# rbesenczi/newMSM

Hardware: AMD Instinct MI355X
Metric: label-cost evals/sec (higher is better)
Workload: dtype f64; 1 GPU; pairwise sulc (D=1) unary label-cost table, ico6 data grid / ico4 control grid, 19 labels, 48678 evals = 3187573 point samples per step (BASELINE config 2); kind=univariate, simmeasure=correlation, replicas=1

## Files before the change

### include/msmhip.h

```cpp
#ifndef MSMHIP_H
#define MSMHIP_H

#include <stddef.h>
#include <stdint.h>

#ifdef __cplusplus
extern "C" {
#endif

#define MSM_ABI_VERSION 12

#define MSM_OK 0
#define MSM_ERR_INVALID (-1)
#define MSM_ERR_HIP (-2)
#define MSM_ERR_OUTSIDE (-3)
#define MSM_ERR_NOTFOUND (-4)
#define MSM_ERR_NOGPU (-5)
#define MSM_ERR_STATE (-6)
#define MSM_ERR_CAPACITY (-7)
#define MSM_ERR_ROTATION (-8)

#define MSM_RAD 100.0
#define MSM_FOLDING 1e7

// ... 3 lines not shown

int         msm_abi_version(void);
const char *msm_last_error(void);
int         msm_device_count(void);

int msm_icosphere_counts(int order, int32_t *V, int32_t *T);
int msm_icosphere(int order, double radius, double *xyz, int32_t *tri);
int msm_mesh_adjacency(const int32_t *tri, int32_t V, int32_t T, int32_t *nbr_ptr, int32_t *nbr, int32_t *tid_ptr, int32_t *tid);
int msm_vertex_areas(const double *xyz, const int32_t *tri, int32_t V, int32_t T, double *area);
int msm_resample_anatomy_grid(const double *cp_xyz, int32_t N, const int32_t *cp_tri, int32_t Tc, int32_t levels, double rad, int32_t *Va, int32_t *Ta,
                              double *axyz, int32_t *atri, int32_t *w_ptr, int32_t *w_cp, double *w_val, int32_t *face_ptr, int32_t *face_idx);
int msm_cp_spacings(const double *xyz, const int32_t *tri, int32_t V, int32_t T, double *maxsep, double *mvdmax);
int msm_label_sampling_grid(int sg_order, double max_dist, int abs_is_int, int32_t cap,
                            double *samples, int32_t *nsamples, double *barycentres, int32_t *nbarycentres);
int msm_rescale_sampling_grid(const double *samples, int32_t n, double *scale, double *labels);
int msm_rotation_matrix(const double ci[3], const double index[3], double R[9]);
int msm_cp_rotations(const double centre[3], const double *cp_xyz, int32_t N, double *rot);
int msm_estimate_triplets(const int32_t *tri, int32_t T, int32_t *triplets);
int msm_estimate_pairs(const int32_t *tri, int32_t V, int32_t T, int32_t *pairs);
int msm_octree_signature(const double *xyz, const int32_t *tri, int32_t V, int32_t T, int64_t stats[5], uint64_t *signature);
int msm_ray_table_check(const double *xyz, const int32_t *tri, int32_t V, int32_t T, int32_t nsamples, uint64_t seed, int64_t report[10]);
int msm_ray_hint_check(const double *xyz, const int32_t *tri, int32_t V, int32_t T, int32_t nsamples, uint64_t seed, int64_t report[8], int32_t *cells,
                       int64_t cells_cap);

msm_ctx *msm_ctx_create(int device);
msm_ctx *msm_ctx_create_on_stream(int device, void *hip_stream);
void     msm_ctx_destroy(msm_ctx *ctx);
int      msm_ctx_synchronize(msm_ctx *ctx);
void    *msm_ctx_stream(msm_ctx *ctx);
void     msm_store_release_i64(int64_t *addr, int64_t value);
int64_t  msm_load_acquire_i64(const int64_t *addr);
int64_t  msm_min_acquire_i64(const int64_t *addr, int32_t n);
int      msm_ctx_wait_stream(msm_ctx *ctx, void *hip_stream);
int      msm_ctx_staging_stats(msm_ctx *ctx, int64_t out[4]);
int      msm_ctx_time_queries(msm_ctx *ctx, int enable);
int      msm_ctx_query_kernel_ms(msm_ctx *ctx, double *ms);
int      msm_query_lanes(int64_t n_queries);
void    *msm_host_alloc(msm_ctx *ctx, size_t bytes);
void     msm_host_free(msm_ctx *ctx, void *p);
int      msm_host_register(msm_ctx *ctx, void *p, size_t bytes);

msm_mesh *msm_mesh_create(msm_ctx *ctx, const double *xyz, int32_t V, const int32_t *tri, int32_t T);
void      msm_mesh_destroy(msm_mesh *m);
int       msm_mesh_update_coords(msm_mesh *m, const double *xyz);
int       msm_mesh_get_coords(msm_mesh *m, double *xyz);
int       msm_mesh_set_features(msm_mesh *m, const double *feat, int32_t D);
// ... 80 lines not shown
int msm_cost_patches(msm_cost *c, int32_t *ngroups, int32_t *ptr, int32_t *idx, int64_t cap);
int msm_cost_absolute_weights(msm_cost *c, double *absw );
int msm_cost_unary_table(msm_cost *c, double *U);
int msm_cost_unary_table_async(msm_cost *c);
int msm_cost_unary_table_fetch(msm_cost *c, double *U);
int msm_cost_unary_batch(msm_cost *c, const int32_t *nodes, const int32_t *labels, int32_t n, double *out);
int msm_cost_triplet_batch(msm_cost *c, const int32_t *triplet, const int32_t *la, const int32_t *lb, const int32_t *lc, int32_t n, double *out);
int msm_cost_triplet_octets(msm_cost *c, const int32_t *labeling, int32_t label, double *E);
int msm_cost_triplet_octets_prefetch(msm_cost *c, const int32_t *labeling, int32_t label, double *E);
int msm_cost_prefetch_stats(msm_cost *c, int64_t *taken, int64_t *dropped);
int msm_cost_pairwise_batch(msm_cost *c, const int32_t *pair, const int32_t *la, const int32_t *lb, int32_t n, double *out);
int msm_cost_pairwise_table(msm_cost *c, double *paircosts);
int msm_cost_triplet_table(msm_cost *c, int32_t t0, int32_t t1, double *tcosts);
int msm_cost_total(msm_cost *c, const int32_t *labeling, double *total, double parts[3]);
int msm_cost_enable_timing(msm_cost *c, int enable);
int msm_cost_kernel_times(msm_cost *c, double *ms, int32_t cap, int32_t *n);
int msm_cost_counters(msm_cost *c, int64_t counters[4]);
#define MSM_ROUTE_UNARY 0
#define MSM_ROUTE_MOVE 1
#define MSM_ROUTE_MOVE_NBLK 2
#define MSM_ROUTE_MOVE_CAP 3
#define MSM_ROUTE_MOVE_MAXTRI 4
#define MSM_ROUTE_MOVE_TAILS 5
#define MSM_UNARY_NONE 0
#define MSM_UNARY_UNIVARIATE 1
#define MSM_UNARY_FLAT 2
#define MSM_UNARY_FEATURES 3
#define MSM_UNARY_MV8 4
#define MSM_UNARY_PW8_4 5
#define MSM_UNARY_PW8_8 6
#define MSM_MOVE_NONE 0
#define MSM_MOVE_FUSED_0 1
#define MSM_MOVE_FUSED_1 2
#define MSM_MOVE_FUSED_2 3
#define MSM_MOVE_FUSED_3 4
#define MSM_MOVE_OCTETS_SAMPLE 5
#define MSM_MOVE_OCTETS_SAMPLE_MV8 6
#define MSM_MOVE_OCTETS_HO 7
#define MSM_MOVE_STRAIN 8
int msm_cost_routes(msm_cost *c, int32_t routes[8]);

typedef struct msm_group msm_group;
typedef struct msm_group_params {
    int32_t simmeasure;
    int32_t fixnan;
    double  lambda, mu, kappa, k_exp, rexp, range;
// ... 75 lines not shown
```

### newmsm_amd/_lib.py

```python
import ctypes as C
import os

_HERE = os.path.dirname(os.path.abspath(__file__))
LIB_PATH = os.environ.get("MSM_LIB_PATH") or os.path.join(_HERE, "libmsmhip.so")

c_dp = C.POINTER(C.c_double)
c_ip = C.POINTER(C.c_int32)
c_lp = C.POINTER(C.c_int64)

MSM_OK = 0
ERR_NAMES = {-1: "MSM_ERR_INVALID", -2: "MSM_ERR_HIP", -3: "MSM_ERR_OUTSIDE", -4: "MSM_ERR_NOTFOUND", -5: "MSM_ERR_NOGPU",
             -6: "MSM_ERR_STATE", -7: "MSM_ERR_CAPACITY", -8: "MSM_ERR_ROTATION"}


class MsmError(RuntimeError):

    def __init__(self, code, message):
        super().__init__("%s (%d): %s" % (ERR_NAMES.get(code, "MSM_ERR"), code, message))
        self.code = code


class GroupParams(C.Structure):
    _fields_ = [("simmeasure", C.c_int32), ("fixnan", C.c_int32), ("lambda_", C.c_double), ("mu", C.c_double),
                ("kappa", C.c_double), ("k_exp", C.c_double), ("rexp", C.c_double), ("range", C.c_double), ("percentile", C.c_double)]
# ... 5 lines not shown
                ("rexp", C.c_double), ("range", C.c_double), ("percentile", C.c_double)]


_VP = C.c_void_p
SIGNATURES = {
    "msm_abi_version": (C.c_int, []),
    "msm_last_error": (C.c_char_p, []),
    "msm_device_count": (C.c_int, []),
    "msm_icosphere_counts": (C.c_int, [C.c_int, c_ip, c_ip]),
    "msm_icosphere": (C.c_int, [C.c_int, C.c_double, c_dp, c_ip]),
    "msm_mesh_adjacency": (C.c_int, [c_ip, C.c_int32, C.c_int32, c_ip, c_ip, c_ip, c_ip]),
    "msm_vertex_areas": (C.c_int, [c_dp, c_ip, C.c_int32, C.c_int32, c_dp]),
    "msm_resample_anatomy_grid": (C.c_int, [c_dp, C.c_int32, c_ip, C.c_int32, C.c_int32, C.c_double, c_ip, c_ip, c_dp, c_ip, c_ip, c_ip, c_dp, c_ip, c_ip]),
    "msm_cp_spacings": (C.c_int, [c_dp, c_ip, C.c_int32, C.c_int32, c_dp, c_dp]),
    "msm_label_sampling_grid": (C.c_int, [C.c_int, C.c_double, C.c_int, C.c_int32, c_dp, c_ip, c_dp, c_ip]),
    "msm_rescale_sampling_grid": (C.c_int, [c_dp, C.c_int32, c_dp, c_dp]),
    "msm_rotation_matrix": (C.c_int, [c_dp, c_dp, c_dp]),
    "msm_cp_rotations": (C.c_int, [c_dp, c_dp, C.c_int32, c_dp]),
    "msm_estimate_triplets": (C.c_int, [c_ip, C.c_int32, c_ip]),
    "msm_estimate_pairs": (C.c_int, [c_ip, C.c_int32, C.c_int32, c_ip]),
    "msm_octree_signature": (C.c_int, [c_dp, c_ip, C.c_int32, C.c_int32, C.POINTER(C.c_int64), C.POINTER(C.c_uint64)]),
    "msm_ray_table_check": (C.c_int, [c_dp, c_ip, C.c_int32, C.c_int32, C.c_int32, C.c_uint64, C.POINTER(C.c_int64)]),
    "msm_ray_hint_check": (C.c_int, [c_dp, c_ip, C.c_int32, C.c_int32, C.c_int32, C.c_uint64, C.POINTER(C.c_int64), c_ip, C.c_int64]),
    "msm_ctx_create": (_VP, [C.c_int]),
    "msm_ctx_create_on_stream": (_VP, [C.c_int, _VP]),
    "msm_ctx_destroy": (None, [_VP]),
    "msm_ctx_synchronize": (C.c_int, [_VP]),
    "msm_ctx_stream": (_VP, [_VP]),
    "msm_store_release_i64": (None, [_VP, C.c_int64]),
    "msm_load_acquire_i64": (C.c_int64, [_VP]),
    "msm_min_acquire_i64": (C.c_int64, [_VP, C.c_int32]),
    "msm_ctx_time_queries": (C.c_int, [_VP, C.c_int]),
    "msm_ctx_query_kernel_ms": (C.c_int, [_VP, c_dp]),
    "msm_query_lanes": (C.c_int, [C.c_int64]),
    "msm_group_context": (_VP, [_VP]),
    "msm_ctx_wait_stream": (C.c_int, [_VP, _VP]),
    "msm_ctx_staging_stats": (C.c_int, [_VP, C.POINTER(C.c_int64)]),
    "msm_host_alloc": (_VP, [_VP, C.c_size_t]),
    "msm_host_free": (None, [_VP, _VP]),
    "msm_host_register": (C.c_int, [_VP, _VP, C.c_size_t]),
    "msm_mesh_create": (_VP, [_VP, c_dp, C.c_int32, c_ip, C.c_int32]),
    "msm_mesh_destroy": (None, [_VP]),
    "msm_mesh_update_coords": (C.c_int, [_VP, c_dp]),
    "msm_mesh_get_coords": (C.c_int, [_VP, c_dp]),
    "msm_mesh_set_features": (C.c_int, [_VP, c_dp, C.c_int32]),
    "msm_mesh_sizes": (C.c_int, [_VP, c_ip, c_ip, c_ip]),
# ... 134 lines not shown
```

### newmsm_amd/api.py

```python
import ctypes as C

import numpy as np

from ._lib import CostParams, MsmError, c_dp, c_ip, c_lp, check, lib

WEIGHTS_PROJECTED = 0
WEIGHTS_RAW = 1
KINDS = dict(univariate=0, multivariate=1, patchwise=2, ho_univariate=3, ho_multivariate=4)


def _soa(points):
    a = np.ascontiguousarray(np.asarray(points, dtype=np.float64).reshape(-1, 3).T)
    return a, a.ctypes.data_as(c_dp)


def _aos(soa, n):
    return np.ascontiguousarray(np.asarray(soa).reshape(3, n).T)


def _tri_soa(tri):
    a = np.ascontiguousarray(np.asarray(tri, dtype=np.int32).reshape(-1, 3).T)
    return a, a.ctypes.data_as(c_ip)


# ... 767 lines not shown
        check(lib().msm_cost_total(self.h, pl, C.byref(tot), parts.ctypes.data_as(c_dp)))
        return tot.value, parts

    def enable_timing(self, on=True):
        check(lib().msm_cost_enable_timing(self.h, int(on)))

    def kernel_times(self):
        ms = np.zeros(64)
        n = C.c_int32()
        check(lib().msm_cost_kernel_times(self.h, ms.ctypes.data_as(c_dp), 64, C.byref(n)))
        return ms[: n.value].copy()

    def counters(self):
        c = (C.c_int64 * 4)()
        check(lib().msm_cost_counters(self.h, c))
        return dict(samples=c[0], unary=c[1], triplet=c[2], pairwise=c[3])

    UNARY_ROUTES = ("none", "univariate", "flat", "features", "mv8", "pw8<4>", "pw8<8>")
    MOVE_ROUTES = ("none", "fused0", "fused1", "fused2", "fused3", "octets_sample", "octets_sample_mv8", "octets_ho", "strain")

    def routes(self):
        r = (C.c_int32 * 8)()
        check(lib().msm_cost_routes(self.h, r))
        return dict(unary=self.UNARY_ROUTES[r[0]], move=self.MOVE_ROUTES[r[1]], move_nblk=r[2], move_cap=r[3], move_maxtri=r[4], move_tails=r[5])


class DiscreteGroupCostFunction:

    def __init__(self, ctx, num_subjects, simmeasure=2, fixnan=False, lambda_=0.1, mu=0.1, kappa=10.0, k_exp=2.0, rexp=2.0, range_=1.0,
                 percentile=0.75):
        from ._lib import GroupParams

        self.ctx = ctx
        self.S = num_subjects
        self.params = GroupParams(simmeasure, int(fixnan), lambda_, mu, kappa, k_exp, rexp, range_, percentile)
        self.h = lib().msm_group_create(ctx.h, C.byref(self.params), num_subjects)
        if not self.h:
            raise MsmError(-1, lib().msm_last_error().decode())
        self._keep = {}

    def close(self):
        if getattr(self, "h", None) and getattr(self.ctx, "h", None):
            lib().msm_group_destroy(self.h)
        self.h = None

    def __del__(self):
        self.close()
# ... 224 lines not shown
```

### newmsm_amd/csrc/cost.cpp

```cpp
#include <algorithm>
#include <chrono>
#include <cmath>
#include <cstdio>
#include <cstdlib>
#include <cstring>

#include "cost_internal.hpp"
#include "host_parallel.hpp"

using namespace msm;

namespace msm {
int ensure_vertex_major(msm_cost *c) {
    if (c->vm_valid) return MSM_OK;
    msm_ctx *ctx = c->ctx;
    const int Ns = c->source->V, D = c->D, R = c->cfw_rows;
    std::vector<double> vm((size_t)Ns * D);
    for (int d = 0; d < D; ++d)
        for (int v = 0; v < Ns; ++v) vm[(size_t)v * D + d] = c->sfeat[(size_t)d * Ns + v];
    MSM_HIP(c->d_sfeat_vm.ensure(vm.size()));
    {
        const int st = upload_staged(ctx, c->d_sfeat_vm.p, vm.data(), sizeof(double) * vm.size());
        if (st) return st;
    }
// ... 175 lines not shown
    u.tfeat = c->target->d_feat.p;
    u.D = c->D;
    u.N = N;
    u.L = c->L;
    u.cp = c->cpgrid->d_xyz.p;
    st = ensure_label_rotations(c);
    if (st) return st;
    u.rnl = c->d_rnl.p;
    u.labels = c->d_labels.p;
    u.src = c->source->d_xyz.p;
    u.Nsrc = c->source->V;
    u.sfeat = c->d_sfeat.p;
    u.cfw = c->cfw.empty() ? nullptr : c->d_cfw.p;
    u.cfw_rows = c->cfw_rows;
    u.pptr = c->d_pptr.p;
    u.pidx = c->d_pidx.p;
    u.order = c->d_order.p;
    u.absw = c->d_absw.p;
    u.pmax = c->pmax;
    u.simmeasure = c->p.simmeasure;
    u.percentile = c->p.percentile;
    u.U = c->d_U.p;
    const size_t nsamp = (size_t)c->L * c->pidx.size();
    MSM_HIP(c->d_tval.ensure(nsamp));
    MSM_HIP(c->d_fix_list.ensure(nsamp));
    MSM_HIP(c->d_fix_pt.ensure(3 * nsamp));
    if (!c->d_fix_count.p) MSM_HIP(c->d_fix_count.zero(unary_fix_counter_words(), ctx->stream));
    if (!c->fix_off_valid) {
        std::vector<uint32_t> off;
        unary_fix_offsets(N, c->L, c->pmax, c->pptr.data(), c->order.data(), off);
        MSM_TRY(c->d_fix_off.upload(off.data(), off.size(), ctx));
        MSM_TRY(ctx_sync(ctx));
        c->fix_off_valid = true;
    }
    MSM_HIP(c->d_queues.ensure(N));
    u.ntri = c->target->T;
    u.tval = c->d_tval.p;
    u.fix_list = c->d_fix_list.p;
    u.fix_pt = c->d_fix_pt.p;
    u.fix_cnt = c->d_fix_count.p;
    u.fix_off = c->d_fix_off.p;
    u.redo_list = c->d_queues.p;
    u.route = &c->route_unary;
    if (c->timing) {
        u.ev_start = c->ev0[c->ev_next];
        u.ev_stop = c->ev1[c->ev_next];
        c->ev_next = (c->ev_next + 1) % (int)c->ev0.size();
        c->ev_count = std::min(c->ev_count + 1, (int)c->ev0.size());
    }
    switch (c->p.kind) {
        case MSM_COST_UNIVARIATE: st = launch_unary_univariate(ctx, u); break;
        case MSM_COST_MULTIVARIATE:
        case MSM_COST_PATCHWISE: {
            {
                st = ensure_vertex_major(c);
                if (st) return st;
                u.sfeat_vm = c->d_sfeat_vm.p;
                u.cfw_vm = c->cfw.empty() ? nullptr : c->d_cfw_vm.p;
            }
// ... 359 lines not shown
    if (!c || !ms || !n) return fail(MSM_ERR_INVALID, "msm_cost_kernel_times: null argument");
    MSM_TRY(drop_ctx_pending(c->ctx));
    MSM_TRY(ctx_sync(c->ctx));
    const int total = (int)c->ev0.size(), cnt = std::min(c->ev_count, (int)cap);
    for (int k = 0; k < cnt; ++k) {
        const int slot = ((c->ev_next - cnt + k) % total + total) % total;
        float f = 0.f;
        MSM_HIP(hipEventElapsedTime(&f, c->ev0[slot], c->ev1[slot]));
        ms[k] = f;
    }
    *n = cnt;
    return MSM_OK;
}

int msm_cost_routes(msm_cost *c, int32_t routes[8]) {
    if (!c || !routes) return fail(MSM_ERR_INVALID, "msm_cost_routes: null argument");
    for (int i = 0; i < 8; ++i) routes[i] = 0;
    routes[MSM_ROUTE_UNARY] = c->route_unary;
    routes[MSM_ROUTE_MOVE] = c->route_move;
    routes[MSM_ROUTE_MOVE_NBLK] = c->move_nblk;
    routes[MSM_ROUTE_MOVE_CAP] = c->move_cap;
    routes[MSM_ROUTE_MOVE_MAXTRI] = c->move_maxtri;
    routes[MSM_ROUTE_MOVE_TAILS] = (int32_t)std::min<int64_t>(c->move_tails, INT32_MAX);
    return MSM_OK;
}

int msm_cost_counters(msm_cost *c, int64_t counters[4]) {
    if (!c || !counters) return fail(MSM_ERR_INVALID, "msm_cost_counters: null argument");
    counters[0] = c->counters[0];
    counters[1] = c->counters[1];
    counters[2] = c->counters[2];
    counters[3] = c->counters[3];
    return MSM_OK;
}


}
```

### newmsm_amd/csrc/cost_internal.hpp

```cpp
#pragma once

#include <vector>

#include "devbuf.hpp"
#include "kernels.hpp"

using msm::DevBuf;

struct msm_cost {
    msm_ctx *ctx = nullptr;
    msm_cost_params p{};
    msm_mesh *target = nullptr, *source = nullptr, *cpgrid = nullptr;
    std::vector<double> orig_xyz;
    std::vector<double> ocp_xyz;
    int D = 0;
    std::vector<double> sfeat;
    DevBuf<double> d_sfeat;
    DevBuf<double> d_sfeat_vm, d_cfw_vm;
    bool vm_valid = false;
    std::vector<double> cfw;
    int cfw_rows = 0;
    DevBuf<double> d_cfw;
    std::vector<double> maxsep;
    double mvdmax = 0;
// ... 20 lines not shown
        int kind = 0;
        int label = 0;
        double *E = nullptr;
        uint64_t epoch = 0;
        std::vector<int32_t> labeling;
        msm::CliqueArgs a;
        msm::MoveArgs m;
        msm::MoveLabels lab;
    } pending;
    int64_t prefetch_hits = 0, prefetch_drops = 0;
    DevBuf<unsigned> d_defer_list, d_defer_cnt;
    int move_nblk = 0, move_cap = 0, move_parity = 0;
    int move_maxtri = 0;
    int route_unary = 0, route_move = 0;
    bool move_valid = false;
    bool have_source = false;
    int ngroups = 0, pmax = 0;
    std::vector<int32_t> pptr, pidx;
    DevBuf<int32_t> d_pptr, d_pidx;
    std::vector<int32_t> order;
    DevBuf<int32_t> d_order;
    DevBuf<uint32_t> d_fix_off;
    bool fix_off_valid = false;
    std::vector<double> absw;
    DevBuf<int32_t> d_pidx_asc;
    DevBuf<uint32_t> d_code;
    DevBuf<double4> d_chunkb;
    bool pidx_asc_on_device = false;
    int patch_cap_hint = 0;
    DevBuf<double> d_absw, d_maxw;
    DevBuf<double> d_U;
    bool table_valid = false;
    bool rotations_valid = false;
    std::vector<double> h_U;
    DevBuf<unsigned long long> d_counters;
    int64_t counters[4] = {0, 0, 0, 0};
    DevBuf<uint32_t> d_slots;
    DevBuf<double> d_tval;
    DevBuf<int> d_stri;
    DevBuf<double> d_sw3;
    DevBuf<unsigned long long> d_fix_list;
    DevBuf<double> d_fix_pt;
    DevBuf<unsigned int> d_fix_count;
    msm_mesh *asphere = nullptr;
    int aVs = 0, aTs = 0;
    DevBuf<double> d_atarget, d_asrc, d_aw_val;
// ... 19 lines not shown
```

### newmsm_amd/csrc/kernels.hpp

```cpp
#pragma once

#include "internal.hpp"

namespace msm {

int launch_build_masks(msm_ctx *ctx, const DevTree &T, const double4 *d_nodebox, unsigned long long *d_mask);
int launch_build_recs(msm_ctx *ctx, const double *d_xyz, int V, const int32_t *d_tri, int T, TriRec *d_rec, float4 *d_tcone, const int32_t *d_leaf_tri,
                      int nentries, float4 *d_cone);
int launch_build_recs_forest(msm_ctx *ctx, const double *d_xyz, size_t comp_stride, size_t tree_stride, const int32_t *d_tri, int T, int B, TriRec *d_rec, float4 *d_tcone,
                             size_t s_rec, const int32_t *d_leaf_tri, float4 *d_cone, size_t s_leaf, const int *d_entries, size_t entries_stride);
int launch_build_raytri(msm_ctx *ctx, const TriRec *d_rec, const float4 *d_edge, int T, const double *d_feat1, int D, float4 *d_out);
struct AdaptiveDevArgs {
    int nOld, nNew;
    const int *fvid, *rvid;
    const double *fw, *rw;
    const double *oldA, *newA;
    int *roff, *rfill, *rkey;
    double *rwt;
    int *coff, *cfill, *ckey;
    double *cval, *correction;
    int *scan_tmp;
    int *long_flag;
    int *tkey;
    double *tval;
// ... 40 lines not shown
struct UnaryLaunch {
    DevTree tree;
    const double *tfeat;
    int D;
    int N, L;
    const double *cp;
    const double *rnl;
    const double *labels;
    const double *src;
    int Nsrc;
    const double *sfeat;
    const double *cfw;
    int cfw_rows;
    const double *sfeat_vm = nullptr;
    const double *cfw_vm = nullptr;
    const int *pptr, *pidx;
    const int *order;
    const double *absw;
    int pmax;
    int simmeasure;
    double percentile;
    double *U;
    int ntri;
    double *tval;
    unsigned long long *fix_list;
    double *fix_pt;
    unsigned int *fix_cnt;
    const unsigned int *fix_off;
    int *redo_list;
    hipEvent_t ev_start = nullptr, ev_stop = nullptr;
    int *route = nullptr;
};
int unary_nsplit(int L, int pmax);
int unary_fix_segments();
size_t unary_fix_counter_words();
void unary_fix_offsets(int N, int L, int pmax, const int32_t *pptr, const int32_t *order, std::vector<uint32_t> &off);
int launch_unary_univariate(msm_ctx *ctx, const UnaryLaunch &u);
struct UnaryWeightsScratch {
    int *stri;
    double *sw3;
};
int launch_unary_multivariate(msm_ctx *ctx, const UnaryLaunch &u, const UnaryWeightsScratch &w, bool patchwise);

struct CliqueArgs {
    int kind, simmeasure;
    int N, L, T, P;
    const int *triplets;
    const int *pairs;
    const double *cp;
    const double *ocp;
    const double *orig;
    int Norig;
    const double *moved;
    const double *rnl;
    const int *cp_tri;
    int Tc;
    const int *cp_tid_ptr, *cp_tid;
    double lambda, mu, kappa, k_exp, rexp, mvdmax, percentile;
    DevTree tree;
// ... 133 lines not shown
```

### newmsm_amd/csrc/unary_kernels.hip

```cpp
#include <algorithm>
#include <cstdlib>

#include "kernels.hpp"
#include "search_device.hpp"
#include "similarity_device.hpp"

#ifndef MSM_VARIANT
#define MSM_VARIANT 0
#endif

namespace msm {

namespace {

constexpr int kFixSegs = 64;
constexpr int kCntStride = 32;
constexpr int kChunk = 768;
constexpr int kQueueCap = 3072;
constexpr int kDeferred = 1 << 20;
constexpr unsigned kInvalidPair = 0xffffffffu;
constexpr int kTriBits = 22;

__device__ __forceinline__ void raise_status(int *status, int code) { atomicMin(status, code); }

__device__ __forceinline__ double wave_sum(double v) {
#pragma unroll
    for (int off = 32; off > 0; off >>= 1) v += __shfl_xor(v, off, 64);
    return v;
}

struct SamplesArgs {
    DevTree tree;
    const double *tfeat;
    int tD;
    int N, L;
    const double *rnl;
    const double *src;
    int Nsrc;
    const int *pptr, *pidx;
    const int *order;
    int pmax;
    int nsplit;
    double *tval;
    int *stri;
    double *sw3;
    unsigned long long *fix_list;
    double *fix_pt;
    unsigned int *fix_cnt;
    const unsigned int *fix_off;
    const double *sfeat;
    const double *cfw;
    const double *absw;
    int simmeasure;
    double percentile;
    double *U;
    int *redo_list;
    unsigned int *redo_count;
    int *status;
};

__device__ __forceinline__ int fast_div(int s, int P, float invP) {
    int q = (int)((float)s * invP);
    if (q * P > s) --q;
    else if ((q + 1) * P <= s) ++q;
    return q;
// ... 235 lines not shown
                    } else {
                        raise_status(a.status, MSM_ERR_CAPACITY);
                    }
                }
            }
            __syncthreads();
#endif
        }
        if (a.U) {
            __syncthreads();
            if (s_ndefer == 0) {
                const double absw = a.absw[node];
                for (int l = l_beg + (tid >> 6); l < l_end; l += 4) {
                    const double cost = patch_similarity(sA, sW, sT + (l - l_beg) * a.pmax, P, lane, a.simmeasure, a.percentile);
                    if (lane == 0) a.U[(size_t)l * a.N + node] = absw * cost;
                }
            } else if (tid == 0) {
                a.redo_list[atomicAdd(a.redo_count, 1u)] = node;
            }
        }
    }
}

__global__ __launch_bounds__(256) void k_unary_rays(SamplesArgs a) {
    extern __shared__ __align__(16) double lds[];
    double *sx = lds, *sy = sx + a.pmax, *sz = sy + a.pmax, *sR = sz + a.pmax;
    const int tid = threadIdx.x, lane = tid & 63;
    const int per = (a.N + 7) >> 3;
    const int slots = 8 * per;
    const int part = blockIdx.x / slots, slot = blockIdx.x - part * slots;
    const int at = (slot & 7) * per + (slot >> 3);
    if (at >= a.N) return;
    const int node = a.order[at];
    const int lper = (a.L + a.nsplit - 1) / a.nsplit;
    const int l_beg = part * lper, l_end = min(a.L, l_beg + lper);
    if (l_beg >= l_end) return;
    const int beg = a.pptr[node], P = a.pptr[node + 1] - beg;
    const size_t gbase = (size_t)a.L * beg;
    for (int i = tid; i < P; i += 256) {
        const int s = a.pidx[beg + i];
        sx[i] = a.src[s];
        sy[i] = a.src[a.Nsrc + s];
        sz[i] = a.src[2 * a.Nsrc + s];
    }
    for (int k = 9 * l_beg + tid; k < 9 * l_end; k += 256) sR[k] = a.rnl[(size_t)node * a.L * 9 + k];
    const int sbeg = l_beg * P, send = l_end * P;
    const float invP = 1.0f / (float)max(P, 1);
    int *sleft = reinterpret_cast<int *>(sR + 9 * a.L);
    __shared__ int s_nleft;
    __shared__ unsigned s_base;
    if (tid == 0) s_nleft = 0;
    __syncthreads();
    for (int s0 = sbeg; s0 < send; s0 += 256) {
        const int s = s0 + tid;
        const bool act = s < send;
        bool done = false;
        V3 p = mk(0.0, 0.0, 0.0);
        float fx = 0.f, fy = 0.f, fz = 0.f;
        int4 c = make_int4(-1, -1, -1, -1);
        if (act) {
            const int l = fast_div(s, P, invP), i = s - l * P;
            p = rotate(sR + 9 * l, mk(sx[i], sy[i], sz[i]));
            c = ray_cell_of(a.tree, p, fx, fy, fz);
        }
        if (act) {
            if (c.x >= 0) {
                const float4 *rec = a.tree.ray_tri + (size_t)kRayPieces * c.x;
                const float4 e0 = rec[0], e1 = rec[1], e2 = rec[2];
                const double2 *dv = reinterpret_cast<const double2 *>(rec + 3);
                double2 d0 = dv[0], d1 = dv[1], d2 = dv[2], d3 = dv[3], d4 = dv[4], d5 = dv[5];
                int t = c.x;
                bool vouch_needed = __float_as_int(e1.w) >= 0;
                float4 ev = e1;
                if (!ray_accepts(e0, e1, e2, fx, fy, fz)) {
                    t = -1;
                    int4 mo = make_int4(c.w, -1, -1, -1);
                    if (c.w < -1) mo = a.tree.ray_more[-2 - c.w];
#pragma unroll 1
                    for (int k = 0; k < 6 && t < 0; ++k) {
                        const int ck = k == 0 ? c.y : (k == 1 ? c.z : (k == 2 ? mo.x : (k == 3 ? mo.y : (k == 4 ? mo.z : mo.w))));
                        if (ck < 0) break;
                        const float4 *r2 = a.tree.ray_tri + (size_t)kRayPieces * ck;
                        const float4 g0 = r2[0], g1 = r2[1], g2 = r2[2];
                        if (ray_accepts(g0, g1, g2, fx, fy, fz)) {
// ... 18 lines not shown
                        a.stri[g] = t;
                        a.sw3[3 * g] = wa;
                        a.sw3[3 * g + 1] = wb;
                        a.sw3[3 * g + 2] = wc;
                    }
                    done = true;
                }
            }
        }
        const bool left = act && !done;
        const unsigned long long bal = __ballot(left);
        if (bal) {
            const int leader = __ffsll((long long)bal) - 1;
            int base = 0;
            if (lane == leader) base = atomicAdd(&s_nleft, __popcll(bal));
            base = __shfl(base, leader, 64);
            if (left) sleft[base + __popcll(bal & ((1ull << lane) - 1ull))] = s;
        }
    }
    __syncthreads();
    const int nleft = s_nleft;
    if (nleft > 0) {
        const int seg = blockIdx.x % kFixSegs;
        if (tid == 0) s_base = a.fix_off[seg] + atomicAdd(&a.fix_cnt[kCntStride * (1 + seg)], (unsigned)nleft);
        __syncthreads();
        const unsigned base = s_base, end = a.fix_off[seg + 1];
        for (int j = tid; j < nleft; j += 256) {
            if (base + j < end) {
                const int s = sleft[j];
                const int l = fast_div(s, P, invP), i = s - l * P;
                const V3 p = rotate(sR + 9 * l, mk(sx[i], sy[i], sz[i]));
                a.fix_list[base + j] = gbase + (unsigned long long)s;
                a.fix_pt[3 * (size_t)(base + j)] = p.x;
                a.fix_pt[3 * (size_t)(base + j) + 1] = p.y;
                a.fix_pt[3 * (size_t)(base + j) + 2] = p.z;
            } else {
                raise_status(a.status, MSM_ERR_CAPACITY);
            }
        }
    }
}

__global__ __launch_bounds__(256) void k_unary_fixup(SamplesArgs a) {
    __shared__ unsigned s_pre[kFixSegs + 1];
    if (threadIdx.x < kFixSegs) {
        const int seg = threadIdx.x;
        const unsigned cnt = min(a.fix_cnt[kCntStride * (1 + seg)], a.fix_off[seg + 1] - a.fix_off[seg]);
        unsigned incl = cnt;
#pragma unroll
        for (int off = 1; off < 64; off <<= 1) {
            const unsigned up = __shfl_up(incl, off, 64);
            if (seg >= off) incl += up;
        }
        s_pre[seg + 1] = incl;
        if (seg == 0) s_pre[0] = 0;
    }
    __syncthreads();
    const unsigned n = s_pre[kFixSegs];
    const int lane = threadIdx.x & 63, sub = lane & 7, grp = lane >> 3;
    const unsigned per_block = 256 / 8, stride = gridDim.x * per_block;
    for (unsigned j0 = blockIdx.x * per_block + (threadIdx.x >> 6) * 8; j0 < n; j0 += stride) {
        const unsigned j = j0 + grp;
        const bool valid = j < n;
// ... 11 lines not shown
        const int found = group8_find(a.tree, valid, p, lane);
        if (valid && sub == 0) {
            const int t = found == kGroupUndecided ? find_closest_triangle(a.tree, p) : found;
            if (t < 0) emit_failure(a, g, t);
            else emit_sample(a, g, p, t);
        }
    }
}

struct ReduceArgs {
    int N, L, Nsrc;
    const double *sfeat;
    const double *cfw;
    int cfw_rows;
    const int *pptr, *pidx;
    const double *absw;
    const double *tval;
    int pmax;
    int simmeasure;
    double percentile;
    double *U;
    const int *redo_list;
    const unsigned int *redo_count;
};

__global__ __launch_bounds__(256) void k_unary_reduce_univariate(ReduceArgs a) {
    extern __shared__ __align__(16) double lds[];
    double *sA = lds, *sW = sA + a.pmax;
    const int tid = threadIdx.x, lane = tid & 63, wave = tid >> 6;
    const unsigned n = a.redo_count ? *a.redo_count : (unsigned)a.N;
    for (unsigned k = blockIdx.x; k < n; k += gridDim.x) {
        const int node = a.redo_list ? a.redo_list[k] : (int)k;
        const int beg = a.pptr[node], P = a.pptr[node + 1] - beg;
        __syncthreads();
        for (int i = tid; i < P; i += 256) {
            const int s = a.pidx[beg + i];
            sA[i] = a.sfeat[s];
            sW[i] = (a.cfw && a.cfw_rows >= 1) ? a.cfw[s] : 1.0;
        }
        __syncthreads();
        const double absw = a.absw[node];
        for (int l = wave; l < a.L; l += 4) {
            const double cost = patch_similarity(sA, sW, a.tval + (size_t)a.L * beg + (size_t)l * P, P, lane, a.simmeasure, a.percentile);
            if (lane == 0) a.U[(size_t)l * a.N + node] = absw * cost;
        }
    }
}

constexpr int kRedLanes = 8;
constexpr int kRedKeep = 12;

__device__ __forceinline__ double group_sum(double v) {
#pragma unroll
    for (int off = kRedLanes / 2; off > 0; off >>= 1) v += __shfl_xor(v, off, kRedLanes);
    return v;
}

__global__ __launch_bounds__(256) void k_unary_reduce_flat(ReduceArgs a, unsigned int *clear, int clear_words) {
    extern __shared__ __align__(16) double lds[];
    double *sA = lds, *sW = sA + a.pmax;
    __shared__ double s_stat[3];
    const int tid = threadIdx.x, sub = tid & (kRedLanes - 1), grp = tid / kRedLanes;
    if (blockIdx.x == 0 && clear)
        for (int k = tid; k < clear_words; k += 256) clear[k] = 0u;
    const int node = a.redo_list ? a.redo_list[blockIdx.x] : (int)blockIdx.x;
    const int beg = a.pptr[node], P = a.pptr[node + 1] - beg;
    const bool has_w = a.cfw && a.cfw_rows >= 1;
    const bool in_regs = true;
    double breg[kRedKeep];
#pragma unroll
    for (int k = 0; k < kRedKeep; ++k) breg[k] = 0.0;
    if (grp < a.L) {
        const double *B = a.tval + (size_t)a.L * beg + (size_t)grp * P;
#pragma unroll
        for (int k = 0; k < kRedKeep; ++k) breg[k] = (sub + kRedLanes * k < P) ? B[sub + kRedLanes * k] : 0.0;
    }
    for (int i = tid; i < P; i += 256) {
        const int s = a.pidx[beg + i];
        sA[i] = a.sfeat[s];
        sW[i] = has_w ? a.cfw[s] : 1.0;
    }
    __syncthreads();
    if (a.simmeasure == 2) {
        if (tid < 64) {
            double sw = 0, ma = 0;
            for (int i = tid; i < P; i += 64) {
                sw += sW[i];
                ma += sW[i] * sA[i];
            }
            sw = wave_sum(sw);
            ma = wave_sum(ma);
            if (sw > 0.0) ma /= sw;
            double va = 0;
            for (int i = tid; i < P; i += 64) {
                const double da = sA[i] - ma;
                va += sW[i] * da * da;
            }
            va = wave_sum(va);
            if (tid == 0) s_stat[0] = sw, s_stat[1] = ma, s_stat[2] = va;
        }
        __syncthreads();
    }
    const double absw = a.absw[node];
    for (int l = grp; l < a.L; l += 256 / kRedLanes) {
        const double *B = a.tval + (size_t)a.L * beg + (size_t)l * P;
        if (!(in_regs && l == grp)) {
#pragma unroll
            for (int k = 0; k < kRedKeep; ++k) breg[k] = (sub + kRedLanes * k < P) ? B[sub + kRedLanes * k] : 0.0;
        }
        double cost;
        if (a.simmeasure == 2) {
            const double sw = s_stat[0], ma = s_stat[1];
            double mb = 0;
#pragma unroll
            for (int k = 0; k < kRedKeep; ++k) {
                const int i = sub + kRedLanes * k;
                if (i < P) mb += sW[i] * breg[k];
            }
            for (int i = sub + kRedLanes * kRedKeep; i < P; i += kRedLanes) mb += sW[i] * B[i];
            mb = group_sum(mb);
            if (sw > 0.0) mb /= sw;
            double pr = 0, vb = 0;
#pragma unroll
            for (int k = 0; k < kRedKeep; ++k) {
                const int i = sub + kRedLanes * k;
                if (i < P) {
                    const double da = sA[i] - ma, db = breg[k] - mb;
                    pr += sW[i] * da * db;
// ... 325 lines not shown
        double total = 0.0;
#pragma unroll
        for (int k = 0; k < K; ++k)
            if (j + kMvLanes * k < D) total += c[k];
        total = mv_group_sum(total);
        double cost = total / D;
        if (__ballot(bad)) cost = nan;
        if (lane == 0) a.U[(size_t)l * a.N + node] = absw * cost;
    }
}

static size_t samples_lds(int pmax, int L, int nsplit) {
    const size_t lper = (size_t)(L + nsplit - 1) / nsplit;
    return sizeof(double) * (5 * (size_t)pmax + 9 * (size_t)L + lper * pmax) + sizeof(unsigned) * kQueueCap + sizeof(int) * 2 * kChunk;
}

int unary_nsplit(int L, int pmax) {
    int n = std::max(1, std::min(4, (int)(((size_t)L * pmax + kChunk - 1) / kChunk)));
    while (n < L && samples_lds(pmax, L, n) > 64 * 1024) ++n;
    return std::min(n, std::max(L, 1));
}
int unary_fix_segments() { return kFixSegs; }
size_t unary_fix_counter_words() { return (size_t)kCntStride * (1 + kFixSegs); }
void unary_fix_offsets(int N, int L, int pmax, const int32_t *pptr, const int32_t *order, std::vector<uint32_t> &off) {
    const int nsplit = unary_nsplit(L, pmax), per = (N + 7) >> 3, slots = 8 * per;
    const int lper = (L + nsplit - 1) / nsplit;
    std::vector<uint64_t> size(kFixSegs, 0);
    for (int b = 0; b < nsplit * slots; ++b) {
        const int part = b / slots, slot = b - part * slots;
        const int at = (slot & 7) * per + (slot >> 3);
        if (at >= N) continue;
        const int node = order[at];
        const int l_beg = part * lper, l_end = std::min(L, l_beg + lper);
        if (l_beg >= l_end) continue;
        size[b % kFixSegs] += (uint64_t)(l_end - l_beg) * (pptr[node + 1] - pptr[node]);
    }
    off.assign(kFixSegs + 1, 0);
    for (int s = 0; s < kFixSegs; ++s) off[s + 1] = (uint32_t)std::min<uint64_t>(0xffffffffull, off[s] + size[s]);
}

static bool uses_ray_table(const DevTree &t) { return t.simple && t.ray_G > 0 && t.ray_cell && t.ray_tri; }

static int launch_samples(msm_ctx *ctx, const UnaryLaunch &u, const UnaryWeightsScratch *w, SamplesArgs &a, bool fused_reduction = false) {
    if (u.tree.nnodes <= 0 || !u.tree.mask) return fail(MSM_ERR_STATE, "target search structure missing");
    a.tree = u.tree;
    a.tfeat = u.tfeat;
    a.tD = u.D > 0 ? u.D : 1;
    a.N = u.N;
    a.L = u.L;
    a.rnl = u.rnl;
    a.src = u.src;
    a.Nsrc = u.Nsrc;
    a.pptr = u.pptr;
    a.pidx = u.pidx;
    a.order = u.order;
    a.pmax = u.pmax;
    a.tval = w ? nullptr : u.tval;
    a.stri = w ? w->stri : nullptr;
    a.sw3 = w ? w->sw3 : nullptr;
    a.fix_list = u.fix_list;
    a.fix_pt = u.fix_pt;
    a.fix_cnt = u.fix_cnt;
    a.fix_off = u.fix_off;
    a.sfeat = u.sfeat;
    a.cfw = (u.cfw && u.cfw_rows >= 1) ? u.cfw : nullptr;
    a.absw = u.absw;
    a.simmeasure = u.simmeasure;
    a.percentile = u.percentile;
    a.U = (w || !fused_reduction) ? nullptr : u.U;
    a.redo_list = u.redo_list;
    a.redo_count = u.fix_cnt;
    a.status = ctx->d_status;
    if (u.ntri >= (1 << kTriBits)) return fail(MSM_ERR_CAPACITY, "target mesh has %d triangles; the sample queue packs ids in %d bits", u.ntri, kTriBits);
    a.nsplit = unary_nsplit(u.L, u.pmax);
    const size_t lds = samples_lds(u.pmax, u.L, a.nsplit);
    if (!uses_ray_table(u.tree) && lds > 64 * 1024) {
        if (lds > 160 * 1024) return fail(MSM_ERR_CAPACITY, "a patch of %d points does not fit in LDS", u.pmax);
        MSM_HIP(hipFuncSetAttribute(reinterpret_cast<const void *>(k_unary_samples), hipFuncAttributeMaxDynamicSharedMemorySize, (int)lds));
    }
    const int blocks = a.nsplit * 8 * ((u.N + 7) / 8);
    if (u.ev_start) MSM_HIP(hipEventRecord(u.ev_start, ctx->stream));
    if (uses_ray_table(u.tree)) {
        a.U = nullptr;
        const int lper = (u.L + a.nsplit - 1) / a.nsplit;
        const size_t rays_lds = sizeof(double) * (3 * (size_t)u.pmax + 9 * (size_t)u.L) + sizeof(int) * ((size_t)lper * u.pmax + 4) + 16;
        if (rays_lds > 64 * 1024) MSM_HIP(hipFuncSetAttribute(reinterpret_cast<const void *>(k_unary_rays), hipFuncAttributeMaxDynamicSharedMemorySize, (int)rays_lds));
        hipLaunchKernelGGL(k_unary_rays, dim3(blocks), dim3(256), rays_lds, ctx->stream, a);
    } else {
        hipLaunchKernelGGL(k_unary_samples, dim3(blocks), dim3(256), lds, ctx->stream, a);
    }
    MSM_HIP(hipGetLastError());
    if (u.ev_stop) MSM_HIP(hipEventRecord(u.ev_stop, ctx->stream));
    hipLaunchKernelGGL(k_unary_fixup, dim3(4096), dim3(256), 0, ctx->stream, a);
    MSM_HIP(hipGetLastError());
    return MSM_OK;
}

int launch_unary_univariate(msm_ctx *ctx, const UnaryLaunch &u) {
    SamplesArgs a;
    const bool dice = u.simmeasure == 4 || u.simmeasure == 5;
    int st = launch_samples(ctx, u, nullptr, a, dice);
    if (st) return st;
    ReduceArgs r;
    r.N = u.N;
    r.L = u.L;
    r.Nsrc = u.Nsrc;
    r.sfeat = u.sfeat;
    r.cfw = u.cfw;
    r.cfw_rows = u.cfw_rows;
    r.pptr = u.pptr;
    r.pidx = u.pidx;
    r.absw = u.absw;
    r.tval = u.tval;
    r.pmax = u.pmax;
    r.simmeasure = u.simmeasure;
    r.percentile = u.percentile;
    r.U = u.U;
    r.redo_list = u.redo_list;
    r.redo_count = u.fix_cnt;
    if (u.route) *u.route = dice ? MSM_UNARY_UNIVARIATE : MSM_UNARY_FLAT;
    if (uses_ray_table(u.tree) && dice) {
        r.redo_list = nullptr;
        r.redo_count = nullptr;
        hipLaunchKernelGGL(k_unary_reduce_univariate, dim3(std::min(u.N, 2048)), dim3(256), sizeof(double) * 2 * (size_t)u.pmax, ctx->stream, r);
        MSM_HIP(hipMemsetAsync(u.fix_cnt, 0, unary_fix_counter_words() * sizeof(unsigned), ctx->stream));
    } else if (!dice) {
        r.redo_list = u.order;
        hipLaunchKernelGGL(k_unary_reduce_flat, dim3(u.N), dim3(256), sizeof(double) * 2 * (size_t)u.pmax, ctx->stream, r, u.fix_cnt,
                           (int)unary_fix_counter_words());
    } else {
        hipLaunchKernelGGL(k_unary_reduce_univariate, dim3(64), dim3(256), sizeof(double) * 2 * (size_t)u.pmax, ctx->stream, r);
        MSM_HIP(hipMemsetAsync(u.fix_cnt, 0, unary_fix_counter_words() * sizeof(unsigned), ctx->stream));
    }
    MSM_HIP(hipGetLastError());
    return MSM_OK;
}

int launch_unary_multivariate(msm_ctx *ctx, const UnaryLaunch &u, const UnaryWeightsScratch &w, bool patchwise) {
    SamplesArgs a;
    int st = launch_samples(ctx, u, &w, a);
    if (st) return st;
    ReduceMvArgs r;
    r.N = u.N;
    r.L = u.L;
    r.Nsrc = u.Nsrc;
    r.D = u.D;
    r.tfeat = u.tfeat;
    r.rec = u.tree.rec;
    r.sfeat = u.sfeat;
    r.cfw = u.cfw;
    r.cfw_rows = u.cfw_rows;
// ... 55 lines not shown
```

Measured before the change: 375.2 million evals/s.

## Skip identity-rotation labels by sampling each source vertex once per step

Adds extra vertex blocks to the ray-table sampling kernel that sample every source vertex once, unrotated, into a shared region appended to the tval buffer. Per-node label blocks then compact away labels whose rotation is exactly identity, so they no longer sample those points. The flat reduction reads the per-vertex values for identity labels instead. With 19 labels, one of which is typically the zero displacement, this cuts roughly a nineteenth of the sampling work. It adds extra LDS, a per-label identity check in the reducer, and a device counter for vertex fixups.

```diff
diff --git a/include/msmhip.h b/include/msmhip.h
--- a/include/msmhip.h
+++ b/include/msmhip.h
@@ -49,6 +49,7 @@
 int msm_ray_table_check(const double *xyz, const int32_t *tri, int32_t V, int32_t T, int32_t nsamples, uint64_t seed, int64_t report[10]);
 int msm_ray_hint_check(const double *xyz, const int32_t *tri, int32_t V, int32_t T, int32_t nsamples, uint64_t seed, int64_t report[8], int32_t *cells,
                        int64_t cells_cap);
+int msm_unary_fix_offsets(int32_t N, int32_t L, int32_t pmax, int32_t Nsrc, const int32_t *pptr, const int32_t *order, uint32_t off[65], int32_t *nsplit);
 
 msm_ctx *msm_ctx_create(int device);
 msm_ctx *msm_ctx_create_on_stream(int device, void *hip_stream);
@@ -175,6 +176,7 @@
 #define MSM_ROUTE_MOVE_CAP 3
 #define MSM_ROUTE_MOVE_MAXTRI 4
 #define MSM_ROUTE_MOVE_TAILS 5
+#define MSM_ROUTE_UNARY_VERTEX_FIXUPS 6
 #define MSM_UNARY_NONE 0
 #define MSM_UNARY_UNIVARIATE 1
 #define MSM_UNARY_FLAT 2
diff --git a/newmsm_amd/_lib.py b/newmsm_amd/_lib.py
--- a/newmsm_amd/_lib.py
+++ b/newmsm_amd/_lib.py
@@ -51,6 +51,7 @@
     "msm_octree_signature": (C.c_int, [c_dp, c_ip, C.c_int32, C.c_int32, C.POINTER(C.c_int64), C.POINTER(C.c_uint64)]),
     "msm_ray_table_check": (C.c_int, [c_dp, c_ip, C.c_int32, C.c_int32, C.c_int32, C.c_uint64, C.POINTER(C.c_int64)]),
     "msm_ray_hint_check": (C.c_int, [c_dp, c_ip, C.c_int32, C.c_int32, C.c_int32, C.c_uint64, C.POINTER(C.c_int64), c_ip, C.c_int64]),
+    "msm_unary_fix_offsets": (C.c_int, [C.c_int32, C.c_int32, C.c_int32, C.c_int32, c_ip, c_ip, C.POINTER(C.c_uint32), c_ip]),
     "msm_ctx_create": (_VP, [C.c_int]),
     "msm_ctx_create_on_stream": (_VP, [C.c_int, _VP]),
     "msm_ctx_destroy": (None, [_VP]),
diff --git a/newmsm_amd/api.py b/newmsm_amd/api.py
--- a/newmsm_amd/api.py
+++ b/newmsm_amd/api.py
@@ -813,7 +813,8 @@
     def routes(self):
         r = (C.c_int32 * 8)()
         check(lib().msm_cost_routes(self.h, r))
-        return dict(unary=self.UNARY_ROUTES[r[0]], move=self.MOVE_ROUTES[r[1]], move_nblk=r[2], move_cap=r[3], move_maxtri=r[4], move_tails=r[5])
+        return dict(unary=self.UNARY_ROUTES[r[0]], move=self.MOVE_ROUTES[r[1]], move_nblk=r[2], move_cap=r[3], move_maxtri=r[4], move_tails=r[5],
+                    unary_vertex_fixups=r[6])
 
 
 class DiscreteGroupCostFunction:
diff --git a/newmsm_amd/csrc/cost.cpp b/newmsm_amd/csrc/cost.cpp
--- a/newmsm_amd/csrc/cost.cpp
+++ b/newmsm_amd/csrc/cost.cpp
@@ -221,19 +221,22 @@
     u.percentile = c->p.percentile;
     u.U = c->d_U.p;
     const size_t nsamp = (size_t)c->L * c->pidx.size();
-    MSM_HIP(c->d_tval.ensure(nsamp));
-    MSM_HIP(c->d_fix_list.ensure(nsamp));
-    MSM_HIP(c->d_fix_pt.ensure(3 * nsamp));
+    MSM_HIP(c->d_tval.ensure(nsamp + (size_t)c->source->V));
     if (!c->d_fix_count.p) MSM_HIP(c->d_fix_count.zero(unary_fix_counter_words(), ctx->stream));
     if (!c->fix_off_valid) {
         std::vector<uint32_t> off;
-        unary_fix_offsets(N, c->L, c->pmax, c->pptr.data(), c->order.data(), off);
+        unary_fix_offsets(N, c->L, c->pmax, c->source->V, c->pptr.data(), c->order.data(), off);
         MSM_TRY(c->d_fix_off.upload(off.data(), off.size(), ctx));
         MSM_TRY(ctx_sync(ctx));
+        c->fix_cap = off.back();
         c->fix_off_valid = true;
     }
+    MSM_HIP(c->d_fix_list.ensure(c->fix_cap));
+    MSM_HIP(c->d_fix_pt.ensure(3 * c->fix_cap));
     MSM_HIP(c->d_queues.ensure(N));
     u.ntri = c->target->T;
+    u.nsamp = nsamp;
+    u.vertex_fixups = c->d_counters.p;
     u.tval = c->d_tval.p;
     u.fix_list = c->d_fix_list.p;
     u.fix_pt = c->d_fix_pt.p;
@@ -639,6 +642,23 @@
     routes[MSM_ROUTE_MOVE_CAP] = c->move_cap;
     routes[MSM_ROUTE_MOVE_MAXTRI] = c->move_maxtri;
     routes[MSM_ROUTE_MOVE_TAILS] = (int32_t)std::min<int64_t>(c->move_tails, INT32_MAX);
+    if (c->route_unary == MSM_UNARY_FLAT && c->d_counters.p) {
+        unsigned long long n = 0;
+        (void)hipSetDevice(c->ctx->device);
+        MSM_HIP(hipMemcpyAsync(&n, c->d_counters.p, sizeof(n), hipMemcpyDeviceToHost, c->ctx->stream));
+        MSM_TRY(ctx_sync(c->ctx));
+        routes[MSM_ROUTE_UNARY_VERTEX_FIXUPS] = (int32_t)std::min<unsigned long long>(n, INT32_MAX);
+    }
+    return MSM_OK;
+}
+
+int msm_unary_fix_offsets(int32_t N, int32_t L, int32_t pmax, int32_t Nsrc, const int32_t *pptr, const int32_t *order, uint32_t off[65], int32_t *nsplit) {
+    if (N < 1 || L < 1 || pmax < 0 || Nsrc < 0 || !pptr || !order || !off) return fail(MSM_ERR_INVALID, "msm_unary_fix_offsets: bad arguments");
+    std::vector<uint32_t> o;
+    unary_fix_offsets(N, L, pmax, Nsrc, pptr, order, o);
+    if ((int)o.size() != unary_fix_segments() + 1 || o.size() != 65) return fail(MSM_ERR_STATE, "msm_unary_fix_offsets: %d segments", (int)o.size() - 1);
+    std::copy(o.begin(), o.end(), off);
+    if (nsplit) *nsplit = unary_nsplit(L, pmax);
     return MSM_OK;
 }
 
diff --git a/newmsm_amd/csrc/cost_internal.hpp b/newmsm_amd/csrc/cost_internal.hpp
--- a/newmsm_amd/csrc/cost_internal.hpp
+++ b/newmsm_amd/csrc/cost_internal.hpp
@@ -66,6 +66,7 @@
     DevBuf<int32_t> d_order;
     DevBuf<uint32_t> d_fix_off;
     bool fix_off_valid = false;
+    size_t fix_cap = 0;
     std::vector<double> absw;
     DevBuf<int32_t> d_pidx_asc;
     DevBuf<uint32_t> d_code;
diff --git a/newmsm_amd/csrc/kernels.hpp b/newmsm_amd/csrc/kernels.hpp
--- a/newmsm_amd/csrc/kernels.hpp
+++ b/newmsm_amd/csrc/kernels.hpp
@@ -86,9 +86,11 @@
     double percentile;
     double *U;
     int ntri;
+    size_t nsamp;
     double *tval;
     unsigned long long *fix_list;
     double *fix_pt;
+    unsigned long long *vertex_fixups = nullptr;
     unsigned int *fix_cnt;
     const unsigned int *fix_off;
     int *redo_list;
@@ -98,7 +100,7 @@
 int unary_nsplit(int L, int pmax);
 int unary_fix_segments();
 size_t unary_fix_counter_words();
-void unary_fix_offsets(int N, int L, int pmax, const int32_t *pptr, const int32_t *order, std::vector<uint32_t> &off);
+void unary_fix_offsets(int N, int L, int pmax, int Nsrc, const int32_t *pptr, const int32_t *order, std::vector<uint32_t> &off);
 int launch_unary_univariate(msm_ctx *ctx, const UnaryLaunch &u);
 struct UnaryWeightsScratch {
     int *stri;
diff --git a/newmsm_amd/csrc/unary_kernels.hip b/newmsm_amd/csrc/unary_kernels.hip
--- a/newmsm_amd/csrc/unary_kernels.hip
+++ b/newmsm_amd/csrc/unary_kernels.hip
@@ -41,6 +41,10 @@
     const int *order;
     int pmax;
     int nsplit;
+    int pst;
+    int skip_identity;
+    size_t vert_off;
+    unsigned long long *vertex_fixups;
     double *tval;
     int *stri;
     double *sw3;
@@ -322,44 +326,88 @@
     }
 }
 
-__global__ __launch_bounds__(256) void k_unary_rays(SamplesArgs a) {
+#ifndef MSM_UNARY_SKIP_IDENTITY
+#define MSM_UNARY_SKIP_IDENTITY 1
+#endif
+
+__device__ __forceinline__ bool is_identity9(const double *R) {
+    const unsigned long long *u = reinterpret_cast<const unsigned long long *>(R);
+    const unsigned long long one = 0x3ff0000000000000ull;
+    return u[0] == one && u[4] == one && u[8] == one && (u[1] | u[2] | u[3] | u[5] | u[6] | u[7]) == 0ull;
+}
+
+template <bool VBLOCK>
+__device__ __forceinline__ void unary_rays_body(const SamplesArgs &a) {
     extern __shared__ __align__(16) double lds[];
-    double *sx = lds, *sy = sx + a.pmax, *sz = sy + a.pmax, *sR = sz + a.pmax;
+    double *sx = lds, *sy = sx + a.pst, *sz = sy + a.pst, *sR = sz + a.pst;
+    int *smap = reinterpret_cast<int *>(sR + 9 * a.L);
+    int *sleft = smap + a.L;
+    __shared__ int s_nleft, s_nlab;
+    __shared__ unsigned s_base;
     const int tid = threadIdx.x, lane = tid & 63;
     const int per = (a.N + 7) >> 3;
     const int slots = 8 * per;
-    const int part = blockIdx.x / slots, slot = blockIdx.x - part * slots;
-    const int at = (slot & 7) * per + (slot >> 3);
-    if (at >= a.N) return;
-    const int node = a.order[at];
-    const int lper = (a.L + a.nsplit - 1) / a.nsplit;
-    const int l_beg = part * lper, l_end = min(a.L, l_beg + lper);
-    if (l_beg >= l_end) return;
-    const int beg = a.pptr[node], P = a.pptr[node + 1] - beg;
-    const size_t gbase = (size_t)a.L * beg;
-    for (int i = tid; i < P; i += 256) {
-        const int s = a.pidx[beg + i];
-        sx[i] = a.src[s];
-        sy[i] = a.src[a.Nsrc + s];
-        sz[i] = a.src[2 * a.Nsrc + s];
-    }
-    for (int k = 9 * l_beg + tid; k < 9 * l_end; k += 256) sR[k] = a.rnl[(size_t)node * a.L * 9 + k];
-    const int sbeg = l_beg * P, send = l_end * P;
-    const float invP = 1.0f / (float)max(P, 1);
-    int *sleft = reinterpret_cast<int *>(sR + 9 * a.L);
-    __shared__ int s_nleft;
-    __shared__ unsigned s_base;
+    int P, l_beg = 0, lper = 1;
+    size_t gbase;
+    if (!VBLOCK) {
+        const int part = blockIdx.x / slots, slot = blockIdx.x - part * slots;
+        const int at = (slot & 7) * per + (slot >> 3);
+        if (at >= a.N) return;
+        const int node = a.order[at];
+        const int beg = a.pptr[node];
+        P = a.pptr[node + 1] - beg;
+        lper = (a.L + a.nsplit - 1) / a.nsplit;
+        l_beg = part * lper;
+        if (l_beg >= a.L) return;
+        gbase = (size_t)a.L * beg;
+        for (int i = tid; i < P; i += 256) {
+            const int s = a.pidx[beg + i];
+            sx[i] = a.src[s];
+            sy[i] = a.src[a.Nsrc + s];
+            sz[i] = a.src[2 * a.Nsrc + s];
+        }
+        const double *R = a.rnl + (size_t)node * a.L * 9;
+        for (int k = tid; k < 9 * a.L; k += 256) sR[k] = R[k];
+        if (tid < 64) {
+            int n = 0;
+            for (int l0 = 0; l0 < a.L; l0 += 64) {
+                const int l = l0 + lane;
+                const bool keep = l < a.L && !(a.skip_identity && is_identity9(R + 9 * l));
+                const unsigned long long bal = __ballot(keep);
+                if (keep) smap[n + __popcll(bal & ((1ull << lane) - 1ull))] = l;
+                n += __popcll(bal);
+            }
+            if (lane == 0) s_nlab = n;
+        }
+    } else {
+        const int v0 = 256 * ((int)blockIdx.x - a.nsplit * slots);
+        P = min(256, a.Nsrc - v0);
+        gbase = a.vert_off + (size_t)v0;
+        if (tid < P) {
+            sx[tid] = a.src[v0 + tid];
+            sy[tid] = a.src[a.Nsrc + v0 + tid];
+            sz[tid] = a.src[2 * a.Nsrc + v0 + tid];
+        }
+        if (tid < 9) sR[tid] = (tid & 3) == 0 ? 1.0 : 0.0;
+        if (tid == 0) s_nlab = 1;
+    }
     if (tid == 0) s_nleft = 0;
     __syncthreads();
+    const int nlab = __builtin_amdgcn_readfirstlane(s_nlab);
+    const int sbeg = l_beg * P, send = max(l_beg, min(nlab, l_beg + lper)) * P;
+    const float invP = 1.0f / (float)max(P, 1);
     for (int s0 = sbeg; s0 < send; s0 += 256) {
-        const int s = s0 + tid;
-        const bool act = s < send;
+        const int sp = s0 + tid;
+        const bool act = sp < send;
         bool done = false;
+        int s = 0;
         V3 p = mk(0.0, 0.0, 0.0);
         float fx = 0.f, fy = 0.f, fz = 0.f;
         int4 c = make_int4(-1, -1, -1, -1);
         if (act) {
-            const int l = fast_div(s, P, invP), i = s - l * P;
+            const int lp = VBLOCK ? 0 : fast_div(sp, P, invP), i = sp - lp * P;
+            const int l = VBLOCK ? 0 : smap[lp];
+            s = l * P + i;
             p = rotate(sR + 9 * l, mk(sx[i], sy[i], sz[i]));
             c = ray_cell_of(a.tree, p, fx, fy, fz);
         }
@@ -424,13 +472,14 @@
     const int nleft = s_nleft;
     if (nleft > 0) {
         const int seg = blockIdx.x % kFixSegs;
+        if (VBLOCK && tid == 0 && a.vertex_fixups) atomicAdd(a.vertex_fixups, (unsigned long long)nleft);
         if (tid == 0) s_base = a.fix_off[seg] + atomicAdd(&a.fix_cnt[kCntStride * (1 + seg)], (unsigned)nleft);
         __syncthreads();
         const unsigned base = s_base, end = a.fix_off[seg + 1];
         for (int j = tid; j < nleft; j += 256) {
             if (base + j < end) {
                 const int s = sleft[j];
-                const int l = fast_div(s, P, invP), i = s - l * P;
+                const int l = VBLOCK ? 0 : fast_div(s, P, invP), i = s - l * P;
                 const V3 p = rotate(sR + 9 * l, mk(sx[i], sy[i], sz[i]));
                 a.fix_list[base + j] = gbase + (unsigned long long)s;
                 a.fix_pt[3 * (size_t)(base + j)] = p.x;
@@ -441,6 +490,11 @@
             }
         }
     }
+}
+
+__global__ __launch_bounds__(256) void k_unary_rays(SamplesArgs a) {
+    if ((int)blockIdx.x < a.nsplit * 8 * ((a.N + 7) >> 3)) unary_rays_body<false>(a);
+    else unary_rays_body<true>(a);
 }
 
 __global__ __launch_bounds__(256) void k_unary_fixup(SamplesArgs a) {
@@ -498,6 +552,9 @@
     double *U;
     const int *redo_list;
     const unsigned int *redo_count;
+    const double *rnl;
+    size_t vert_off;
+    int skip_identity;
 };
 
 __global__ __launch_bounds__(256) void k_unary_reduce_univariate(ReduceArgs a) {
@@ -535,6 +592,7 @@
 __global__ __launch_bounds__(256) void k_unary_reduce_flat(ReduceArgs a, unsigned int *clear, int clear_words) {
     extern __shared__ __align__(16) double lds[];
     double *sA = lds, *sW = sA + a.pmax;
+    double *sV = sW + a.pmax;
     __shared__ double s_stat[3];
     const int tid = threadIdx.x, sub = tid & (kRedLanes - 1), grp = tid / kRedLanes;
     if (blockIdx.x == 0 && clear)
@@ -546,6 +604,14 @@
     double breg[kRedKeep];
 #pragma unroll
     for (int k = 0; k < kRedKeep; ++k) breg[k] = 0.0;
+    auto identity_label = [&](int l) {
+        if (!a.skip_identity) return false;
+        const unsigned long long *u = reinterpret_cast<const unsigned long long *>(a.rnl + ((size_t)node * a.L + l) * 9);
+        const unsigned long long one = 0x3ff0000000000000ull;
+        bool ok = u[sub] == ((sub & 3) == 0 ? one : 0ull);
+        if (sub == 0) ok = ok && u[8] == one;
+        return ((__ballot(ok) >> (tid & 56)) & 0xffull) == 0xffull;
+    };
     if (grp < a.L) {
         const double *B = a.tval + (size_t)a.L * beg + (size_t)grp * P;
 #pragma unroll
@@ -555,8 +621,14 @@
         const int s = a.pidx[beg + i];
         sA[i] = a.sfeat[s];
         sW[i] = has_w ? a.cfw[s] : 1.0;
-    }
+        if (a.skip_identity) sV[i] = a.tval[a.vert_off + s];
+    }
+    const bool ident0 = grp < a.L && identity_label(grp);
     __syncthreads();
+    if (ident0) {
+#pragma unroll
+        for (int k = 0; k < kRedKeep; ++k) breg[k] = (sub + kRedLanes * k < P) ? sV[sub + kRedLanes * k] : 0.0;
+    }
     if (a.simmeasure == 2) {
         if (tid < 64) {
             double sw = 0, ma = 0;
@@ -579,7 +651,8 @@
     }
     const double absw = a.absw[node];
     for (int l = grp; l < a.L; l += 256 / kRedLanes) {
-        const double *B = a.tval + (size_t)a.L * beg + (size_t)l * P;
+        const bool ident = l == grp ? ident0 : identity_label(l);
+        const double *B = ident ? sV : a.tval + (size_t)a.L * beg + (size_t)l * P;
         if (!(in_regs && l == grp)) {
 #pragma unroll
             for (int k = 0; k < kRedKeep; ++k) breg[k] = (sub + kRedLanes * k < P) ? B[sub + kRedLanes * k] : 0.0;
@@ -951,7 +1024,7 @@
 }
 int unary_fix_segments() { return kFixSegs; }
 size_t unary_fix_counter_words() { return (size_t)kCntStride * (1 + kFixSegs); }
-void unary_fix_offsets(int N, int L, int pmax, const int32_t *pptr, const int32_t *order, std::vector<uint32_t> &off) {
+void unary_fix_offsets(int N, int L, int pmax, int Nsrc, const int32_t *pptr, const int32_t *order, std::vector<uint32_t> &off) {
     const int nsplit = unary_nsplit(L, pmax), per = (N + 7) >> 3, slots = 8 * per;
     const int lper = (L + nsplit - 1) / nsplit;
     std::vector<uint64_t> size(kFixSegs, 0);
@@ -960,10 +1033,11 @@
         const int at = (slot & 7) * per + (slot >> 3);
         if (at >= N) continue;
         const int node = order[at];
+        const int P = pptr[node + 1] - pptr[node];
         const int l_beg = part * lper, l_end = std::min(L, l_beg + lper);
-        if (l_beg >= l_end) continue;
-        size[b % kFixSegs] += (uint64_t)(l_end - l_beg) * (pptr[node + 1] - pptr[node]);
-    }
+        if (l_beg < l_end) size[b % kFixSegs] += (uint64_t)(l_end - l_beg) * P;
+    }
+    for (int v0 = 0, b = nsplit * slots; v0 < Nsrc; v0 += 256, ++b) size[b % kFixSegs] += (uint64_t)std::min(256, Nsrc - v0);
     off.assign(kFixSegs + 1, 0);
     for (int s = 0; s < kFixSegs; ++s) off[s + 1] = (uint32_t)std::min<uint64_t>(0xffffffffull, off[s] + size[s]);
 }
@@ -1002,6 +1076,10 @@
     a.status = ctx->d_status;
     if (u.ntri >= (1 << kTriBits)) return fail(MSM_ERR_CAPACITY, "target mesh has %d triangles; the sample queue packs ids in %d bits", u.ntri, kTriBits);
     a.nsplit = unary_nsplit(u.L, u.pmax);
+    a.pst = u.pmax;
+    a.skip_identity = 0;
+    a.vert_off = u.nsamp;
+    a.vertex_fixups = u.vertex_fixups;
     const size_t lds = samples_lds(u.pmax, u.L, a.nsplit);
     if (!uses_ray_table(u.tree) && lds > 64 * 1024) {
         if (lds > 160 * 1024) return fail(MSM_ERR_CAPACITY, "a patch of %d points does not fit in LDS", u.pmax);
@@ -1011,10 +1089,13 @@
     if (u.ev_start) MSM_HIP(hipEventRecord(u.ev_start, ctx->stream));
     if (uses_ray_table(u.tree)) {
         a.U = nullptr;
-        const int lper = (u.L + a.nsplit - 1) / a.nsplit;
-        const size_t rays_lds = sizeof(double) * (3 * (size_t)u.pmax + 9 * (size_t)u.L) + sizeof(int) * ((size_t)lper * u.pmax + 4) + 16;
+        a.skip_identity = (MSM_UNARY_SKIP_IDENTITY && !w && !fused_reduction) ? 1 : 0;
+        const int vblocks = a.skip_identity ? (u.Nsrc + 255) / 256 : 0;
+        if (vblocks) a.pst = std::max(u.pmax, 256);
+        const size_t left_cap = std::max<size_t>((size_t)((u.L + a.nsplit - 1) / a.nsplit) * u.pmax, vblocks ? 256 : 0);
+        const size_t rays_lds = sizeof(double) * (3 * (size_t)a.pst + 9 * (size_t)u.L) + sizeof(int) * ((size_t)u.L + left_cap + 4) + 16;
         if (rays_lds > 64 * 1024) MSM_HIP(hipFuncSetAttribute(reinterpret_cast<const void *>(k_unary_rays), hipFuncAttributeMaxDynamicSharedMemorySize, (int)rays_lds));
-        hipLaunchKernelGGL(k_unary_rays, dim3(blocks), dim3(256), rays_lds, ctx->stream, a);
+        hipLaunchKernelGGL(k_unary_rays, dim3(blocks + vblocks), dim3(256), rays_lds, ctx->stream, a);
     } else {
         hipLaunchKernelGGL(k_unary_samples, dim3(blocks), dim3(256), lds, ctx->stream, a);
     }
@@ -1047,6 +1128,9 @@
     r.U = u.U;
     r.redo_list = u.redo_list;
     r.redo_count = u.fix_cnt;
+    r.rnl = u.rnl;
+    r.vert_off = u.nsamp;
+    r.skip_identity = a.skip_identity;
     if (u.route) *u.route = dice ? MSM_UNARY_UNIVARIATE : MSM_UNARY_FLAT;
     if (uses_ray_table(u.tree) && dice) {
         r.redo_list = nullptr;
@@ -1055,7 +1139,7 @@
         MSM_HIP(hipMemsetAsync(u.fix_cnt, 0, unary_fix_counter_words() * sizeof(unsigned), ctx->stream));
     } else if (!dice) {
         r.redo_list = u.order;
-        hipLaunchKernelGGL(k_unary_reduce_flat, dim3(u.N), dim3(256), sizeof(double) * 2 * (size_t)u.pmax, ctx->stream, r, u.fix_cnt,
+        hipLaunchKernelGGL(k_unary_reduce_flat, dim3(u.N), dim3(256), sizeof(double) * (r.skip_identity ? 3 : 2) * (size_t)u.pmax, ctx->stream, r, u.fix_cnt,
                            (int)unary_fix_counter_words());
     } else {
         hipLaunchKernelGGL(k_unary_reduce_univariate, dim3(64), dim3(256), sizeof(double) * 2 * (size_t)u.pmax, ctx->stream, r);
```

Result: slower. 357.7 million evals/s (-4.7%).
